# edsonportosilva/OptiCommPy

Hardware: AMD Instinct MI355X
Metric: SSFM steps/sec (2-pol, 2^20 samples) (higher is better)
Workload: dtype f64

## Files before the change

### opticommpy_amd/csrc/fused_engine.h

```cpp
#pragma once
#include <algorithm>
#include <cmath>
#include <cstdlib>
#include <cstring>
#include <memory>
#include <string>
#include <type_traits>
#include <vector>

#include "fused_kernels.h"
#include "ssf_derived.h"

namespace ssf {
namespace fused {

#ifndef SSF_EXPERIMENTS
#define SSF_EXPERIMENTS 0
#endif
static inline const char *tune_env(const char *name) {
#if SSF_EXPERIMENTS
    return std::getenv(name);
#else
    (void)name;
    return nullptr;
// ... 101 lines not shown
            if (force_c && C != force_c) continue;
            const size_t cl = mix2_col_lds(n1, C, 2, s), rl = 4096 + (size_t)n2 * s;
            if (cl > 156 * 1024) continue;
            double score = (cl <= 80 * 1024 ? 0.0 : 4.0) + ((rl <= 72 * 1024 && n2 <= 4096) ? 0.0 : 3.0) + (C == 8 ? 0.0 : C == 4 ? 1.0 : 3.0) +
                           0.5 * std::fabs(std::log2((double)n1 / 256.0));
            const double col_wgs = (double)((n2 + C - 1) / C), row_wgs = (2 * n1 >= 1024 && n2 <= 2048) ? (double)n1 : 2.0 * n1;
            score += 4.0 * std::max(0.0, std::log2(256.0 / col_wgs)) + 4.0 * std::max(0.0, std::log2(256.0 / row_wgs));
            MixPlan cp;
            const int tcol = 256 / (2 * C);
            if (mix_make_plan(n1, &cp, tcol, false))
                for (int i = 0; i < cp.npass; ++i) score += 0.5 * (double)((n1 / cp.r[i] + tcol - 1) / tcol - 1);
            if (score < best) {
                best = score;
                *N1o = n1;
                *N2o = (int)n2;
                *Co = C;
            }
        }
    }
    return best < 1e300;
}

static inline bool choose_nonpow2_split(int64_t N, int precision, int f1, int fc, bool l1_forced, int *l1, int *N1, int *N2, int *C) {
    *l1 = *N1 = *N2 = *C = 0;
    if (f1 > 0 && choose_mixed2_split(N, precision, N1, N2, C, f1, fc)) return true;
    if (!choose_mixed_split(N, precision, l1, N2)) {
        *l1 = *N2 = 0;
        return choose_mixed2_split(N, precision, N1, N2, C);
    }
    if (*l1 < 7 && !l1_forced) {
        int n1 = 0, n2 = 0, c = 0;
        if (choose_mixed2_split(N, precision, &n1, &n2, &c)) {
            *l1 = 0;
            *N1 = n1;
            *N2 = n2;
            *C = c;
        }
    }
    return true;
}

template <typename T, class Backend> class FusedCore {
  public:
    using C = cx<T>;
    using S = scalar_t<T>;
    static constexpr bool kPacked = sizeof(T) != sizeof(S);
    Backend &be;
    int64_t N;
    int nrows, log2N;
    Split sp;
    int N2mix = 0;
    int mix_rows = 1;
    MixPlan mix_plan{};
    cx<double> *wtab = nullptr;
    int N1mix = 0, mix_cols = 0;
    MixPlan mix_plan1{};
    cx<double> *wtab1 = nullptr;
    int n1() const { return N1mix ? N1mix : 1 << sp.l1; }
    int row_tw_off = 0;
    size_t field_bytes;
    C *G = nullptr, *T0 = nullptr, *T1 = nullptr, *Ehd = nullptr, *noise_d = nullptr;
    S *P = nullptr, *Theta = nullptr;
    bool own_G = true;
    void *cpl_comm = nullptr;
    double *cpl_work = nullptr;
    std::unique_ptr<FusedCore<pf2, Backend>> pk;
    bool use_packed = true;
    bool lim0_bound = true;
    Ctrl *ctrl = nullptr;
    LinOp *linops = nullptr;
    unsigned *gbar = nullptr;
    double *part = nullptr;
    double *tr_hz = nullptr, *tr_lim = nullptr;
    int *tr_it = nullptr;
    long long tr_cap = 0;
    int tr_maxIter = 0;
    std::vector<C *> snaps;
    int row_v = 16;
    int col_v = 16;
    bool underfilled = false;
    int lanes_hint = 1;
    int col_split = 1;
    int row_pair = -1;
    bool split_ok = true;
    int split_penalty = 0;
    static constexpr int kSplitPenalty = 8;
    int hint_n_it = 0;
    int cur = 0;
    unsigned seq = 0;
    int row_block, row_grid, col_block_mk, col_grid_mk, col_block_1, col_grid_1, npart_max;
    size_t row_lds, col_lds_mk, col_lds_1;
    std::string err;

    std::vector<ssf_stats> ustats;
    int units = 1;
    int npairs() const { return kPacked ? nrows : std::max(nrows / 2, 1); }
    int rows_u() const { return nrows / units; }
    int pairs_u() const { return std::max(npairs() / units, 1); }
    FusedCore(Backend &b, int64_t N_, int nrows_, int precision, void *borrowed_G = nullptr, int units_ = 1)
        : be(b), N(N_), nrows(nrows_), units(units_ > 0 ? units_ : 1) {
        if (borrowed_G) {
            G = (C *)borrowed_G;
            own_G = false;
        }
        log2N = 0;
        while ((1ll << log2N) < N) ++log2N;
        if ((N & (N - 1)) == 0) {
            choose_split(log2N, precision, &sp, kPacked);
        } else {
            sp.l1 = sp.l2 = 0;
            int f1 = 0, fc = 0;
            if (const char *e = tune_env("SSF_MIX2")) {
                f1 = std::atoi(e);
                if (const char *q = std::strchr(e, ',')) fc = std::atoi(q + 1);
            }
            if (!choose_nonpow2_split(N, precision, f1, fc, tune_env("SSF_MIX_L1") != nullptr, &sp.l1, &N1mix, &N2mix, &mix_cols))
                sp.l1 = N1mix = N2mix = mix_cols = 0;
        }
        field_bytes = sizeof(C) * (size_t)N * (size_t)nrows;
    }

    void col_geometry(int groups, int npol, int *block, int *grid, size_t *lds) const {
        if (N1mix) {
            *block = 256;
            *grid = groups * ((N2mix + mix_cols - 1) / mix_cols);
            *lds = mix2_col_lds(N1mix, mix_cols, npol, (int)sizeof(C));
            return;
        }
        const int tpf = (1 << sp.l1) / col_v, N2 = N2mix ? N2mix : 1 << sp.l2;
        int half = col_v == 8 ? 512 / npol : 256;
        if (const char *e = tune_env("SSF_COL_HALF")) {
            const int h = std::atoi(e);
            if (h >= tpf && h <= 512 && (h & (h - 1)) == 0) half = h;
        }
        while (half / tpf > N2 && half > tpf) half >>= 1;
        auto wgs = [&](int h) { return (long long)groups * (N2 / (h / tpf)); };
        while (!tune_env("SSF_COL_HALF") && half > 64 &&
               ((wgs(half) < 512 && (half / tpf) * sizeof(C) > 128) || (wgs(half) < 256 && (half / tpf) * sizeof(C) > 64)))
            half >>= 1;
        const int Cc = half / tpf;
        *block = half * npol;
        *grid = groups * ((N2 + Cc - 1) / Cc);
        *lds = std::max((size_t)npol * Cc * lds_col_stride(1 << sp.l1, Cc, (int)sizeof(C)) * sizeof(C), (size_t)half * npol * 16 + 1024);
    }

    int init() {
        if (const char *e = tune_env("SSF_LIM0_BOUND")) lim0_bound = std::atoi(e) != 0;
        if (const char *e = tune_env("SSF_COL_SPLIT")) col_split = std::atoi(e);
        if (const char *e = tune_env("SSF_ROW_PAIR")) row_pair = std::atoi(e) != 0;
        underfilled = (double)rows_u() * (double)N <= 1048576.0;
        col_v = underfilled && sp.l1 != 7 ? 8 : 16;
        if (const char *e = tune_env("SSF_COL_V")) col_v = std::atoi(e) == 8 ? 8 : 16;
        if (N2mix || sp.l1 < 6 || sp.l1 > 10) col_v = 16;
        if (N1mix && !mix_make_plan(N1mix, &mix_plan1, 256 / (2 * mix_cols), false)) {
            err = "fused engine: no pass plan for the column length";
            return SSF_ERR_UNSUPPORTED;
        }
        if (const char *e = N1mix ? tune_env("SSF_MIX_PLAN1") : nullptr) {
            int r[kMixMaxPass], n = 0;
            for (const char *q = e; *q && n < kMixMaxPass;) {
                r[n++] = std::atoi(q);
                while (*q && *q != ',') ++q;
                if (*q == ',') ++q;
            }
            MixPlan mp;
            if (mix_plan_from_radices(N1mix, r, n, &mp)) mix_plan1 = mp;
        }
        const int64_t nfft = (int64_t)rows_u() * n1();
        if (N2mix) {
            int tpr = 128;
            if (const char *e = tune_env("SSF_MIX_TPR")) tpr = std::max(64, std::min(1024, std::atoi(e)));
            while (16 * tpr < N2mix) tpr *= 2;
            mix_rows = std::max(1, 256 / tpr);
            while (nfft % mix_rows) mix_rows >>= 1;
            while (mix_rows > 1 && 4096 + (size_t)mix_rows * N2mix * sizeof(C) > 72 * 1024) mix_rows >>= 1;
            while (mix_rows > 1 && nfft / mix_rows < 512) {
                mix_rows >>= 1;
                tpr *= 2;
            }
            row_block = tpr * mix_rows;
            row_grid = (int)(nfft / mix_rows);
            row_lds = 4096 + (size_t)mix_rows * N2mix * sizeof(C);
            mix_make_plan(N2mix, &mix_plan, tpr);
            if (const char *e = tune_env("SSF_MIX_PLAN")) {
                int r[kMixMaxPass], n = 0;
                for (const char *q = e; *q && n < kMixMaxPass;) {
                    r[n++] = std::atoi(q);
                    while (*q && *q != ',') ++q;
                    if (*q == ',') ++q;
                }
                MixPlan mp;
                if (mix_plan_from_radices(N2mix, r, n, &mp) && mp.r[mp.npass - 1] <= kMixMaxOpRadix) mix_plan = mp;
            }
        } else {
            row_v = underfilled ? 8 : 16;
            if (const char *e = tune_env("SSF_ROW_V")) row_v = std::atoi(e) == 8 ? 8 : 16;
            if (sp.l2 < 6) row_v = 16;
            const int tpf2 = (1 << sp.l2) / row_v, wg = row_v == 8 ? 512 : 256;
            int fpw = tpf2 >= wg ? 1 : wg / tpf2;
            if (underfilled && row_v == 8) fpw = units > 1 ? std::max(1, std::min(fpw, 256 / std::max(tpf2, 1))) : 1;
            if (const char *e = tune_env("SSF_ROW_FPW")) fpw = std::max(1, std::min(fpw, std::atoi(e)));
            while (nfft % fpw) fpw >>= 1;
            row_block = fpw * tpf2;
            row_grid = (int)(nfft / fpw);
            row_lds = std::max((size_t)fpw * lds_slots_per_fft(1 << sp.l2) * sizeof(C), (size_t)row_block * 16 + 2048);
            if ((SSF_TW_TAB & 1) && sizeof(S) == 4) {
                row_tw_off = (int)((row_lds + 15) / 16 * 16);
                row_lds = (size_t)row_tw_off + kTwLdsBytes;
            }
        }
        if (const char *e = std::getenv("SSF_C64_PACKED")) use_packed = std::atoi(e) != 0;
        col_geometry(pairs_u(), kPacked ? 1 : 2, &col_block_mk, &col_grid_mk, &col_lds_mk);
        col_geometry(rows_u(), 1, &col_block_1, &col_grid_1, &col_lds_1);
        npart_max = std::max(col_grid_mk, col_grid_1);
        if (own_G && !(G = (C *)be.alloc(field_bytes))) return oom();
        if (!(T0 = (C *)be.alloc(field_bytes))) return oom();
        if (kPacked && mk_buffers()) return SSF_ERR_OOM;
        if (!(ctrl = (Ctrl *)be.alloc(2 * (size_t)units * sizeof(Ctrl)))) return oom();
        if (!(linops = (LinOp *)be.alloc(2 * sizeof(LinOp)))) return oom();
        if (!(gbar = (unsigned *)be.alloc(8 * sizeof(unsigned)))) return oom();
        if (!(part = (double *)be.alloc(sizeof(double) * 5 * (size_t)units * (size_t)npart_max))) return oom();
        if (N2mix) {
            if (!(wtab = (cx<double> *)be.alloc(sizeof(cx<double>) * (size_t)N2mix))) return oom();
            std::vector<cx<double>> w((size_t)N2mix);
            for (int q = 0; q < N2mix; ++q) {
                const double a = -2.0 * 3.14159265358979323846 * (double)q / (double)N2mix;
                w[(size_t)q].re = std::cos(a);
                w[(size_t)q].im = std::sin(a);
            }
            be.h2d(wtab, w.data(), sizeof(cx<double>) * (size_t)N2mix);
        }
        if (N1mix) {
// ... 254 lines not shown
                    a.bar = gbar;
                    int rc = be.launch_nlse_span(a, pgrid, plds);
                    if (rc) return hiperr();
                }
            } else if (nsteps >= 1) {
                launch_col_plain(CM_NLSE_FIRST, E, (S)0);
                launch_row_lin(linops + 0);
                for (int s = 1; s < nsteps; ++s) {
                    launch_col_plain(CM_NLSE_STEP, E, (S)(p.gamma * p.hz));
                    launch_row_lin(linops + 1);
                }
                launch_col_plain(CM_NLSE_STEP, E, (S)(p.gamma * p.hz));
                launch_row_lin(linops + 0);
                launch_col_plain(CM_NLSE_LAST, E, (S)0);
            }
            int rc = amp_fwd(p, d, span, span - s0, noise, std::exp(d.alpha_lin / 2 * nsteps * p.hz));
            if (rc) return rc;
            if (wants_snapshot(p, span) && (rc = snapshot())) return rc;
            st->steps += nsteps;
            st->transforms += (int64_t)nrows * (2 * (int64_t)nsteps + 2);
        }
        be.sync();
        if (pgrid > 0) {
            unsigned flags[3] = {0, 0, 0};
            be.d2h(flags, gbar, sizeof(flags));
            if (flags[2]) {
                err = "persistent span kernel: grid barrier timed out (workgroups not co-resident?)";
                return SSF_ERR_STATE;
            }
        }
        return be.ok() ? SSF_OK : hiperr();
    }

    MkConst mk_const(const ssf_params &p, const Derived &d) const {
        MkConst k{};
        k.Lspan = p.Lspan;
        k.hz_fixed = p.hz;
        k.tol = p.tol;
        k.maxRot = p.maxNlinPhaseRot;
        k.c8g = d.c8g;
        k.sgn = p.direction >= 0 ? 1.0 : -1.0;
        k.lin_a = d.lin_a;
        k.lin_b = d.lin_b;
        k.w2 = (d.w_scale / (double)N) * (d.w_scale / (double)N);
        k.invN = 1.0 / (double)N;
        k.maxIter = p.maxIter;
        k.adaptive = p.nlprMethod ? 1 : 0;
        k.exact_lim0 = (p.maxIter == 1 || !lim0_bound) ? 1 : 0;
        k.log2N = log2N;
        k.trace_cap = tr_cap;
        k.tr_hz = tr_hz;
        k.tr_it = tr_it;
        k.tr_lim = tr_lim;
        return k;
    }
    void launch_mk_row(const MkConst &k, bool pair = false) {
        RowArgs<T> a = row_args();
        a.use_ctrl = 1;
        a.pair = pair ? 1 : 0;
        a.cin = ctrl + (size_t)(seq & 1) * units;
        a.cout = ctrl + (size_t)((seq + 1) & 1) * units;
        a.k = k;
        const size_t ps = (size_t)units * (size_t)npart_max;
        a.pmax = part;
        a.pnum = part + ps;
        a.pden = part + 2 * ps;
        a.pnum0 = part + 3 * ps;
        a.pden0 = part + 4 * ps;
        a.npart = col_grid_mk;
        if constexpr (Backend::kCanCouple) {
            if (cpl_comm) {
                if (be.couple(cpl_comm, part, ps, col_grid_mk, cpl_work)) return;
                a.pnum0 = cpl_work;
                a.pden0 = cpl_work + 1;
                a.pnum = cpl_work + 2;
                a.pden = cpl_work + 3;
                a.pmax = cpl_work + 4;
                a.npart = 1;
            }
        }
        be.launch_row(a, row_grid, row_block, row_lds, units);
        ++seq;
    }
    void launch_mk_col(const MkConst &k, int mode, int sg = SG_ALL) {
        ColArgs<T> a = col_args(kPacked ? 1 : 2, mode);
        a.sg = sg;
        a.cin = ctrl + (size_t)(seq & 1) * units;
        a.cout = ctrl + (size_t)((seq + 1) & 1) * units;
        a.k = k;
        a.npart = col_grid_mk;
        be.launch_col(a, col_grid_mk, col_block_mk, col_lds_mk, units);
        ++seq;
    }
    int prepare_trace(ssf_trace *trace, int maxIter) {
        const long long cap = trace ? trace->capacity : 0;
        if (cap > tr_cap || maxIter != tr_maxIter) {
            for (void *q : {(void *)tr_hz, (void *)tr_lim, (void *)tr_it})
                if (q) be.free(q);
            tr_hz = tr_lim = nullptr;
            tr_it = nullptr;
            tr_cap = 0;
            if (cap > 0) {
                tr_hz = (double *)be.alloc(sizeof(double) * (size_t)cap);
                tr_it = (int *)be.alloc(sizeof(int) * (size_t)cap);
                tr_lim = (double *)be.alloc(sizeof(double) * (size_t)cap * (size_t)maxIter);
                if (!tr_hz || !tr_it || !tr_lim) return oom();
                tr_cap = cap;
                tr_maxIter = maxIter;
            }
        }
        if (tr_cap > 0) be.memset(tr_lim, 0xFF, sizeof(double) * (size_t)tr_cap * (size_t)maxIter);
        return SSF_OK;
    }

    struct SpanRun {
        long long trace_n = 0;
        double avg_it = 3.0;
        int n_it = 0;
    };
    int run_span(const ssf_params &p, const MkConst &k, SpanRun &sr, ssf_stats *st) {
        std::vector<Ctrl> cs((size_t)units);
        for (auto &c : cs) {
            c = Ctrl{};
            c.state = ST_NEED_S;
            c.cur = cur;
            c.trace_n = sr.trace_n;
        }
        const size_t cbytes = sizeof(Ctrl) * (size_t)units;
        be.h2d(ctrl + (size_t)(seq & 1) * units, cs.data(), cbytes);
        bool persisted = false;
        if constexpr (Backend::kCanPersist && !kPacked) {
            const int workers = be.persist_mk_workers();
            if (workers > 0 && units == 1 && !N2mix && row_block == 256 && col_block_mk == 256 && row_v == 16 && col_v == 16 &&
                std::is_same<T, double>::value) {
                SpanMkArgs<T> a{};
                a.row = row_args();
                a.row.use_ctrl = 1;
                a.row.k = k;
                a.row.pmax = part;
                a.row.pnum = part + npart_max;
                a.row.pden = part + 2 * (size_t)npart_max;
                a.row.pnum0 = part + 3 * (size_t)npart_max;
                a.row.pden0 = part + 4 * (size_t)npart_max;
                a.row.npart = col_grid_mk;
                a.col = col_args(2, CM_MK);
                a.row.tw_off = 0;
                a.col.k = k;
                a.col.npart = col_grid_mk;
                a.ctrl = ctrl;
                a.seq0 = seq;
                a.row_grid = row_grid;
                a.col_grid = col_grid_mk;
                a.max_stages = 1 << 20;
                a.nworkers = std::min(workers, std::max(row_grid, col_grid_mk));
                a.xcd = be.persist_mk_xcd() ? 0 : -1;
                a.ctrl_lds = (std::max(row_lds, col_lds_mk) + 15) / 16 * 16;
                a.bar = gbar;
                const int grid = a.xcd >= 0 ? 8 * a.nworkers : a.nworkers;
                if (be.launch_mk_span(a, grid, a.ctrl_lds + sizeof(Ctrl) + 64)) return hiperr();
                unsigned flags[8] = {0, 0, 0, 0, 0, 0, 0, 0};
                be.d2h(flags, gbar, sizeof(flags));
                if (!be.ok()) return hiperr();
                if (flags[2]) {
                    err = "persistent Manakov kernel: grid barrier timed out (workgroups not co-resident / not on one XCD?)";
                    return SSF_ERR_STATE;
                }
                seq = (seq & ~1u) | (flags[4] & 1u);
                be.d2h(cs.data(), ctrl + (seq & 1), sizeof(Ctrl));
                if (!be.ok()) return hiperr();
                if (cs[0].state != ST_SPAN_DONE || cs[0].pend0) {
                    err = "persistent Manakov kernel: span not finished";
                    return SSF_ERR_STATE;
                }
                persisted = true;
            }
        }
        if (!persisted) {
        launch_mk_col(k, CM_MK);
        int guard = 0;
        long long prev_steps = 0, prev_iters = 0, prev_rare = 0;
        const bool can_split = col_split && split_penalty == 0 && units == 1 && !cpl_comm &&
                               be.can_split_cols(col_args(kPacked ? 1 : 2, CM_MK), col_block_mk);
        bool general_chunk = false;
        int stalls = 0, pos = 0;
        const bool can_pair = can_split && units == 1 && std::is_same<T, double>::value && !N1mix && !N2mix && row_v == 16 && !p.nlprMethod &&
                              PairRows<Backend>::ok(be, sp.l2, row_block) && (row_pair < 0 ? !underfilled : row_pair != 0);
        bool skip_row = false;
        double z_sim = 0.0;
        long long idle_pairs = 0;
        for (;;) {
            double steps_rem = 0.0;
            for (const Ctrl &c : cs) {
                double r;
                if (c.state == ST_SPAN_DONE && !c.pend0) r = 0.0;
                else if (c.steps == 0 && c.state == ST_NEED_S) r = p.nlprMethod ? 8.0 : std::ceil(p.Lspan / p.hz);
                else r = std::max(1.0, std::ceil((p.Lspan - c.z) / (c.hz > 0 ? c.hz : p.hz)));
                steps_rem = std::max(steps_rem, r);
            }
            const bool use_split = can_split && split_ok && !general_chunk;
            const int n_pred = std::max(1, std::min(p.maxIter, sr.n_it > 0 ? sr.n_it : (int)std::lround(sr.avg_it)));
            double est = p.nlprMethod ? steps_rem * (1.0 + sr.avg_it) * 0.6
                                      : steps_rem * (1.0 + (use_split ? std::max((double)n_pred, sr.avg_it) : sr.avg_it)) + 3.0;
            int chunk = (int)std::min(512.0, std::max(2.0, std::ceil(est)));
            if (can_split && split_ok && general_chunk) chunk = std::min(chunk, 8);
            else if (use_split && sr.n_it == 0) chunk = std::min(chunk, 4 * (n_pred + 1));
            const bool pairing = use_split && can_pair;
            z_sim = cs[0].z;
            skip_row = pairing && pos == 0 && cs[0].state == ST_NEED_H;
            for (int i = 0; i < chunk; ++i) {
                if (!(pairing && pos == 0 && skip_row)) launch_mk_row(k, pairing);
                int sg = SG_ALL;
                if (use_split) {
                    sg = pos == 0 ? (SG_H | SG_RARE) : pos < n_pred ? SG_ADV : SG_FIN;
                    if (pairing && pos >= n_pred) {
                        const double hz_sim = pick_hz(k, z_sim, 0.0);
                        skip_row = z_sim + hz_sim < k.Lspan && pick_hz(k, z_sim + hz_sim, 0.0) == hz_sim;
                        z_sim += hz_sim;
                    }
                    pos = pos >= n_pred ? 0 : pos + 1;
                }
                launch_mk_col(k, CM_MK, sg);
            }
            be.d2h(cs.data(), ctrl + (size_t)(seq & 1) * units, cbytes);
            if (!be.ok()) return hiperr();
            long long steps = 0, iters = 0, rare = 0;
            bool done = true;
            double worst = 0.0;
            for (const Ctrl &c : cs) {
                steps += c.steps;
                iters += c.iterations;
                rare += c.n_rebuilt + c.n_recovered;
                done = done && c.state == ST_SPAN_DONE && !c.pend0;
                if (c.steps > 0) worst = std::max(worst, (double)c.iterations / (double)c.steps);
            }
            if (steps > prev_steps) {
                sr.avg_it = units == 1 ? (double)(iters - prev_iters) / (double)(steps - prev_steps) : worst;
                sr.n_it = cs[0].last_nit;
            }
            if (can_split && split_ok && !done) {
                idle_pairs = steps == prev_steps ? idle_pairs + chunk : 0;
                const bool stuck = idle_pairs >= 2 * (n_pred + 1) + 2;
                if (general_chunk && !stuck) general_chunk = false;
                else if (stuck) {
                    general_chunk = true;
                    if (++stalls >= 2) split_ok = false;
                }
                if (rare - prev_rare > (steps - prev_steps) / 4 + 2) split_ok = false;
                if (!split_ok) split_penalty = kSplitPenalty;
            }
            prev_steps = steps;
            prev_iters = iters;
            prev_rare = rare;
            if (done) break;
            if (++guard > (1 << 22)) {
                err = "fused engine: span did not terminate";
                return SSF_ERR_STATE;
            }
        }
        }
        if (units == 1) {
            cur = cs[0].cur;
        } else {
            const size_t ub = sizeof(C) * (size_t)rows_u() * (size_t)N;
            for (int u = 0; u < units; ++u)
                if (cs[(size_t)u].cur != cur)
                    be.d2d((char *)(cur ? T1 : T0) + (size_t)u * ub, (char *)(cur ? T0 : T1) + (size_t)u * ub, ub);
        }
        sr.trace_n = cs[0].trace_n;
        if ((int)ustats.size() != units) ustats.assign((size_t)units, ssf_stats{});
        for (int u = 0; u < units; ++u) {
            const Ctrl &c = cs[(size_t)u];
            ssf_stats &us = ustats[(size_t)u];
            us.steps += c.steps;
            us.iterations += c.iterations;
            us.nonconverged_steps += c.nonconv;
            us.decided_ahead += c.n_ahead;
            us.rebuilt_iterates += c.n_rebuilt;
            us.recovered_fields += c.n_recovered;
            us.transforms += (int64_t)(kPacked ? 2 * rows_u() : rows_u()) * (2 * c.steps + 2 * c.iterations);
        }
        for (const Ctrl &c : cs) {
            st->steps += c.steps;
            st->iterations += c.iterations;
            st->nonconverged_steps += c.nonconv;
            st->decided_ahead += c.n_ahead;
            st->rebuilt_iterates += c.n_rebuilt;
            st->recovered_fields += c.n_recovered;
            st->transforms += (int64_t)(kPacked ? 2 * rows_u() : rows_u()) * (2 * c.steps + 2 * c.iterations);
        }
        return SSF_OK;
    }
    int fetch_trace(ssf_trace *trace, long long trace_n, int maxIter) {
        if (trace) {
            trace->count = trace_n;
            const long long n = std::min(trace_n, (long long)trace->capacity);
            if (n > 0) {
                if (trace->hz) be.d2h(trace->hz, tr_hz, sizeof(double) * (size_t)n);
                if (trace->iters) be.d2h(trace->iters, tr_it, sizeof(int) * (size_t)n);
                if (trace->lims) be.d2h(trace->lims, tr_lim, sizeof(double) * (size_t)n * (size_t)maxIter);
            }
        }
        return be.ok() ? SSF_OK : hiperr();
    }
    MkConst mk_const_for(const ssf_params &p, const Derived &d, ssf_trace *trace) const {
// ... 123 lines not shown
```

### opticommpy_amd/csrc/fused_kernels.h

```cpp
#pragma once
#include "fused_core.h"
#include "mixed_fft.h"
#include "ssf_rng.h"

namespace ssf {
namespace fused {

enum {
    ST_NEED_S = 0,
    ST_AFTER_S = 1,
    ST_NEED_H = 2,
    ST_ROW_ITER = 3,
    ST_NEED_I = 4,
    ST_SPAN_DONE = 6,
    ST_REDO0 = 7,
    ST_RECOVER_A = 8,
    ST_RECOVER_ROW = 9,
    ST_RECOVER_B = 10
};

struct LinOp {
    double cth;
    double mag;
    double Cre[9], Cim[9];
// ... 836 lines not shown
            }
            if (lin16) lb = lin16_bases<V>(cth_pre, k1r + ((long long)rev_pos(p, reg_pos(p, last, br, 0)) << a.log2N1), log2N);
            ctx.issue_fence();
        }
#endif
        fft_dif<-1, V, kTab>(ctx, p, br, v, l, tws);
        ctx.mark(2);
        if (a.prio) ctx.template setprio<1>();
        if (!a.use_ctrl && !a.lin) {
            if (a.fwd_only) {
#pragma unroll
                for (int idx = 0; idx < V; ++idx) g[reg_pos(p, last, br, idx)] = v[idx];
                return;
            }
            const cx<T> *h = a.harr + ((size_t)k1r << a.log2N2);
#pragma unroll
            for (int idx = 0; idx < V; ++idx) v[idx] = v[idx] * h[reg_pos(p, last, br, idx)];
        } else if (p.lg(last) == lgV) {
#if SSF_EARLY_BASES
            if (lo.cth != lb.cth) lb = lin16_bases<V>(lo.cth, k1r + ((long long)rev_pos(p, reg_pos(p, last, br, 0)) << a.log2N1), log2N);
            apply_lin16<V>(lo, lb, v);
#else
            if constexpr (kPair) apply_lin16<V>(lo, lbr, v);
            else {
                const long long k0 = k1r + ((long long)rev_pos(p, reg_pos(p, last, br, 0)) << a.log2N1);
                apply_lin16<V>(lo, k0, log2N, v);
            }
#endif
        } else {
#pragma unroll
            for (int idx = 0; idx < V; ++idx) {
                const long long k = k1r + ((long long)rev_pos(p, reg_pos(p, last, br, idx)) << a.log2N1);
                v[idx] = mul_by_d(v[idx], lin_at(lo, k, log2N));
            }
        }
        ctx.mark(3);
        fft_dit<+1, V, kTab>(ctx, p, br, v, l, tws);
        if (a.prio) ctx.template setprio<0>();
        ctx.mark(4);
        row_store<V>(ctx, a, gdst, p, fr, br, v);
        if constexpr (!kPair) break;
        else {
            if (round || !rp.on) break;
            lo = a.cin->lin;
            lo.mag *= (double)row_n1(a);
            uniform_linop(lo);
            gdst = a.G;
        }
    }
    ctx.mark(5);
    ctx.flush(0);
}

enum {
    CM_NLSE_FIRST = 0,
    CM_NLSE_STEP = 1,
    CM_NLSE_LAST = 2,
    CM_MK = 3,
    CM_PLAIN_FWD = 5,
    CM_PLAIN_INV = 6
};

template <typename T> struct ColArgs {
    cx<T> *G;
    cx<T> *T0, *T1;
    cx<T> *Ehd;
    scalar_t<T> *P;
    scalar_t<T> *Theta;
    int log2N1, log2N2, npol, mode;
    int ngroups;
    scalar_t<T> g_hz;
    const Ctrl *cin;
    Ctrl *cout;
    MkConst k;
    double *pmax, *pnum, *pden, *pnum0, *pden0;
    int npart;
    int N2;
    long long N;
    int vpt;
    long long u_elems;
    int u_part;
    int prio;
    int sg;
    int N1mix, mix_cols;
    MixPlan plan1;
    const cx<double> *wtab1;
};

template <typename T> SSF_HD RowArgs<T> unit_view(const RowArgs<T> &a, int u) {
    RowArgs<T> b = a;
    b.G += (long long)u * a.u_elems;
    if (a.cin) b.cin += u;
    if (a.cout) b.cout += u;
    const long long po = (long long)u * a.u_part;
    if (a.pmax) b.pmax += po;
    if (a.pnum) b.pnum += po;
    if (a.pden) b.pden += po;
    if (a.pnum0) b.pnum0 += po;
    if (a.pden0) b.pden0 += po;
    return b;
}
template <typename T> SSF_HD ColArgs<T> unit_view(const ColArgs<T> &a, int u) {
    ColArgs<T> b = a;
    if (u > 0) {
        const long long fo = (long long)u * a.u_elems;
        b.G += fo;
        if (a.T0) b.T0 += fo;
        if (a.T1) b.T1 += fo;
        if (a.Ehd) b.Ehd += fo;
        const long long N = a.N2 ? a.N : 1ll << (a.log2N1 + a.log2N2);
        if (a.P) b.P += 2 * N * a.ngroups * (long long)u;
        if (a.Theta) b.Theta += N * a.ngroups * (long long)u;
        if (a.cin) b.cin += u;
        if (a.cout) b.cout += u;
        const long long po = (long long)u * a.u_part;
        if (a.pmax) b.pmax += po;
        if (a.pnum) b.pnum += po;
        if (a.pden) b.pden += po;
        if (a.pnum0) b.pnum0 += po;
        if (a.pden0) b.pden0 += po;
    }
    return b;
}

template <typename T, int LG, class Ctx, bool RAGGED = false, int V = 16> struct ColGeom {
    static constexpr int kV = V;
    static constexpr bool kDppT = SSF_PAIR_DPP && V == 16 && sizeof(T) == 8;
    bool dpp;
    PassPlan p;
    int half, pol, t, C, c, b, n2, N2;
    bool valid;
    long long N;
    long long rowbase;
    long long pbase;
    SSF_HD ColGeom(Ctx &ctx, const ColArgs<T> &a) {
        p = make_plan(LG > 0 ? LG : a.log2N1, V == 16 ? 4 : 3);
        half = ctx.nthreads / a.npol;
        dpp = kDppT && a.npol == 2;
        if (kDppT && a.npol == 2) {
            pol = ctx.tid & 1;
            t = ctx.tid >> 1;
        } else {
            pol = ctx.tid / half;
            t = ctx.tid - pol * half;
        }
        C = half / p.tpf;
        c = t % C;
        b = t / C;
        N2 = RAGGED ? a.N2 : 1 << a.log2N2;
        const int tpp = RAGGED ? (N2 + C - 1) / C : N2 / C;
        const int grp = ctx.bid / tpp;
        int tile = ctx.bid - grp * tpp;
        if (tpp % 8 == 0) tile = (tile & 7) * (tpp >> 3) + (tile >> 3);
        else if (RAGGED && tpp > 8) {
            const int q = tpp >> 3, r = tpp & 7, x = tile & 7;
            tile = x * q + (x < r ? x : r) + (tile >> 3);
        }
        n2 = tile * C + c;
        valid = !RAGGED || n2 < N2;
        N = RAGGED ? a.N : 1ll << (a.log2N1 + a.log2N2);
        rowbase = (long long)(grp * a.npol + pol) * N;
        pbase = (long long)grp * N;
    }
    SSF_HD long long freq_off(int q) const { return (long long)(b + p.tpf * q) * N2 + n2; }
    SSF_HD long long time_off(int idx) const {
        return (long long)rev_pos(p, reg_pos(p, p.npass - 1, b, idx)) * N2 + n2;
// ... 21 lines not shown
            w0 = cis2pi<double>((double)SIGN * ((double)(((long long)g.n2 * g.b) % g.N) / (double)g.N));
            ws = cis2pi<double>((double)SIGN * ((double)(((long long)g.n2 * g.p.tpf) % g.N) / (double)g.N));
        } else {
            const long long N = 1ll << log2N;
            w0 = cis2pi<double>((double)SIGN * scale_pow2((double)(((long long)g.n2 * g.b) & (N - 1)), log2N));
            ws = cis2pi<double>((double)SIGN * scale_pow2((double)(((long long)g.n2 * g.p.tpf) & (N - 1)), log2N));
        }
        if (SSF_TW_REUSE) {
            gt.w0 = SIGN > 0 ? w0 : conj(w0);
            gt.ws = SIGN > 0 ? ws : conj(ws);
            gt.have = true;
        }
    }
    constexpr int V = G::kV;
    cx<double> t[V];
    const cx<double> s2 = ws * ws, s4 = s2 * s2;
    t[0] = w0;
    t[1] = w0 * ws;
    t[2] = t[0] * s2;
    t[3] = t[1] * s2;
#pragma unroll
    for (int q = 0; q < 4; ++q) t[4 + q] = t[q] * s4;
    if constexpr (V == 16) {
        const cx<double> s8 = s4 * s4;
#pragma unroll
        for (int q = 0; q < 8; ++q) t[8 + q] = t[q] * s8;
    }
#pragma unroll
    for (int q = 0; q < V; ++q) v[q] = mul_by_d(v[q], t[q]);
}

template <typename U, class Ctx, class G> SSF_HD void pair_swap(Ctx &ctx, const G &g, const U *mine, U *other, U *sh) {
    constexpr int V = G::kV;
    if constexpr (G::kDppT) {
        if (g.dpp) {
#pragma unroll
            for (int idx = 0; idx < V; ++idx) other[idx] = (U)ctx.xchg((double)mine[idx]);
            return;
        }
    }
#pragma unroll
    for (int idx = 0; idx < V; ++idx) sh[(size_t)(g.pol * V + idx) * g.half + g.t] = mine[idx];
    ctx.sync();
#pragma unroll
    for (int idx = 0; idx < V; ++idx) other[idx] = sh[(size_t)((g.pol ^ 1) * V + idx) * g.half + g.t];
}

template <class G> SSF_HD int own_idx(const G &g, int j) { return g.pol ? j + G::kV / 2 : j; }
template <class G> SSF_HD int oth_idx(const G &g, int j) { return g.pol ? j : j + G::kV / 2; }
template <class G> SSF_HD long long own_time_off(const G &g, int j) { return g.pol ? g.time_off(j + G::kV / 2) : g.time_off(j); }
template <typename U, class G> SSF_HD U pick16(const G &g, int idx, const U *own, const U *oth) {
    constexpr int H = G::kV / 2;
    return ((idx / H) == g.pol) ? own[idx % H] : oth[idx % H];
}

template <typename T, class Ctx, class G>
SSF_HD void pair_cis(Ctx &ctx, const G &g, const T *ang_own, cx<T> *rot, cx<T> *sh) {
    constexpr int V = G::kV, H = V / 2;
    cx<T> own[H], oth[H];
    if constexpr (G::kDppT) {
        if (g.dpp) {
#pragma unroll
            for (int j = 0; j < H; ++j) {
                own[j] = cis_t<T>(ang_own[j]);
                oth[j] = mk<T>((T)ctx.xchg((double)own[j].re), (T)ctx.xchg((double)own[j].im));
            }
#pragma unroll
            for (int idx = 0; idx < V; ++idx) rot[idx] = pick16(g, idx, own, oth);
            return;
        }
    }
#pragma unroll
    for (int j = 0; j < H; ++j) {
        own[j] = cis_t<T>(ang_own[j]);
        sh[(size_t)own_idx(g, j) * g.half + g.t] = own[j];
    }
    ctx.sync();
#pragma unroll
    for (int j = 0; j < H; ++j) oth[j] = sh[(size_t)oth_idx(g, j) * g.half + g.t];
#pragma unroll
    for (int idx = 0; idx < V; ++idx) rot[idx] = pick16(g, idx, own, oth);
}

template <typename T, class Ctx, class G>
SSF_HD void mk_step_start(Ctx &ctx, const G &g, const ColArgs<T> &a, const cx<T> *v, T *Pbuf, bool lds_busy) {
    constexpr int V = G::kV;
    T *shT = (T *)ctx.lds;
    T mine[V], oth[V];
#pragma unroll
    for (int idx = 0; idx < V; ++idx) mine[idx] = norm2(v[idx]);
    if (lds_busy && !(G::kDppT && g.dpp)) ctx.sync();
    pair_swap(ctx, g, mine, oth, shT);
    const T c8g = (T)a.k.c8g;
    double m = -INFINITY;
#pragma unroll
    for (int idx = 0; idx < V; ++idx) {
        const T ax = g.pol ? oth[idx] : mine[idx], ay = g.pol ? mine[idx] : oth[idx];
        const T pw = ax + ay;
        if (g.pol == 0) g.st(Pbuf, g.pbase + g.time_off(idx), pw);
        const T phi = c8g * (pw + ax + ay) / (T)2;
        m = (double)phi > m ? (double)phi : m;
    }
    if (a.k.adaptive) {
        m = block_max(ctx, m, (double *)ctx.lds);
        if (ctx.tid == 0) a.pmax[ctx.bid] = m;
    }
    ctx.sync();
}
template <typename T, class G> SSF_HD T theta_ld(const G &g, const T *th, long long i) {
    if constexpr (SSF_THETA_F32 && sizeof(T) == 8) return (T)g.ld((const float *)th, i);
    else return g.ld(th, i);
}
template <typename T, class G> SSF_HD void theta_st(const G &g, T *th, long long i, T x) {
    if constexpr (SSF_THETA_F32 && sizeof(T) == 8) g.st((float *)th, i, (float)x);
    else g.st(th, i, x);
}
template <typename T, class Ctx, class G>
SSF_HD void mk_advance_dpp(Ctx &ctx, const G &g, const ColArgs<T> &a, cx<T> *v, const T *Pbuf, T shz, bool first,
                           double &num, double &den, double &pch_sum) {
    constexpr int V = G::kV, H = V / 2;
    T pw8[H], prev8[H], ang8[H];
#pragma unroll
    for (int j = 0; j < H; ++j) {
        const long long t = own_time_off(g, j);
        pw8[j] = g.ld(Pbuf, g.pbase + t);
        prev8[j] = first ? (T)0 : theta_ld(g, a.Theta, g.pbase + t);
    }
    const T c8g = (T)a.k.c8g;
#pragma unroll
    for (int j = 0; j < H; ++j) {
        const T lo = norm2(v[j]), hi = norm2(v[j + H]);
        const T nown = g.pol ? hi : lo, noth = g.pol ? lo : hi;
        const T po = (T)ctx.xchg((double)noth);
        const T ax = g.pol ? po : nown, ay = g.pol ? nown : po;
        const T pw = pw8[j];
        pch_sum += (double)pw;
        ang8[j] = shz * (c8g * (pw + ax + ay) / (T)2);
        if (first) prev8[j] = shz * (c8g * (pw + pw) / (T)2);
    }
    ctx.mark(6);
#pragma unroll
    for (int idx = 0; idx < V; ++idx) v[idx] = g.ld(a.Ehd, g.rowbase + g.time_off(idx));
    ctx.mark(7);
#pragma unroll
    for (int j = 0; j < H; ++j) {
        const T ang = ang8[j];
        const double s = sin_half_angle((double)ang - (double)prev8[j]);
        theta_st(g, a.Theta, g.pbase + own_time_off(g, j), ang);
        const cx<T> ro = cis_t<T>(ang);
        const T dd = (T)(4.0 * s * s);
        const cx<T> rp = mk<T>((T)ctx.xchg((double)ro.re), (T)ctx.xchg((double)ro.im));
        const T dp = (T)ctx.xchg((double)dd);
        const cx<T> r_lo = g.pol ? rp : ro, r_hi = g.pol ? ro : rp;
        const T d_lo = g.pol ? dp : dd, d_hi = g.pol ? dd : dp;
        const double w0 = (double)norm2(v[j]), w1 = (double)norm2(v[j + H]);
        num += w0 * (double)d_lo + w1 * (double)d_hi;
        den += w0 + w1;
        v[j] = v[j] * r_lo;
        v[j + H] = v[j + H] * r_hi;
    }
}
template <typename T, class Ctx, class G>
SSF_HD void mk_advance(Ctx &ctx, const G &g, const ColArgs<T> &a, cx<T> *v, const T *Pbuf, T shz, bool first,
                       double &num, double &den, double &pch_sum) {
    constexpr int V = G::kV, H = V / 2;
    T *shN = (T *)ctx.lds;
    cx<T> *shC = (cx<T> *)(shN + V * (size_t)g.half);
    T *shD = (T *)(shC + V * (size_t)g.half);
    T nown[H], noth[H];
    T pw8[H], prev8[H];
#pragma unroll
    for (int j = 0; j < H; ++j) {
        const long long t = own_time_off(g, j);
        pw8[j] = g.ld(Pbuf, g.pbase + t);
        prev8[j] = first ? (T)0 : theta_ld(g, a.Theta, g.pbase + t);
    }
#pragma unroll
    for (int j = 0; j < H; ++j) {
        const T lo = norm2(v[j]), hi = norm2(v[j + H]);
        nown[j] = g.pol ? hi : lo;
        noth[j] = g.pol ? lo : hi;
    }
    ctx.sync();
#pragma unroll
    for (int j = 0; j < H; ++j) shN[(size_t)oth_idx(g, j) * g.half + g.t] = noth[j];
    ctx.sync();
    const T c8g = (T)a.k.c8g;
    T ang8[H];
#pragma unroll
    for (int j = 0; j < H; ++j) {
        const T po = shN[(size_t)own_idx(g, j) * g.half + g.t];
        const T ax = g.pol ? po : nown[j], ay = g.pol ? nown[j] : po;
        const T pw = pw8[j];
        pch_sum += (double)pw;
        ang8[j] = shz * (c8g * (pw + ax + ay) / (T)2);
        if (first) prev8[j] = shz * (c8g * (pw + pw) / (T)2);
    }
    ctx.mark(6);
#pragma unroll
    for (int idx = 0; idx < H; ++idx) v[idx] = g.ld(a.Ehd, g.rowbase + g.time_off(idx));
#pragma unroll
    for (int j = 0; j < H; ++j) {
        const long long t = own_time_off(g, j);
        const T ang = ang8[j], prev = prev8[j];
        const double s = sin_half_angle((double)ang - (double)prev);
        theta_st(g, a.Theta, g.pbase + t, ang);
        shC[(size_t)own_idx(g, j) * g.half + g.t] = cis_t<T>(ang);
        shD[(size_t)own_idx(g, j) * g.half + g.t] = (T)(4.0 * s * s);
    }
    ctx.mark(7);
#pragma unroll
    for (int idx = H; idx < V; ++idx) v[idx] = g.ld(a.Ehd, g.rowbase + g.time_off(idx));
    ctx.sync();
#pragma unroll
    for (int idx = 0; idx < V; ++idx) {
        const cx<T> e = v[idx];
        const double w = (double)norm2(e);
        num += w * (double)shD[(size_t)idx * g.half + g.t];
        den += w;
        v[idx] = e * shC[(size_t)idx * g.half + g.t];
    }
    ctx.sync();
}

struct MkColStage {
    bool do_inv = false, do_fwd = false, final_ = false, more = false, exact0 = true;
    bool sparse = false;
    bool paired = false;
    int op = -1;
    struct { int state, it, cur, pcur; double z, hz; } c{};
};
template <int V> SSF_HD bool lim0_bound_sample(int idx, int b) { return idx == 0 && (V == 16 || !(b & 1)); }
enum { SG_H = 1, SG_ADV = 2, SG_FIN = 4, SG_RARE = 8, SG_ALL = 15 };
SSF_HD int stage_group(int op, bool final_) { return op == 1 ? SG_H : op == 2 ? (final_ ? SG_FIN : SG_ADV) : SG_RARE; }
template <class Ctx, class Args> SSF_HD void mk_col_stage(Ctx &ctx, const Args &a, MkColStage &st, int sg_mask = SG_ALL) {
    bool &do_inv = st.do_inv, &do_fwd = st.do_fwd, &final_ = st.final_, &more = st.more, &exact0 = st.exact0;
    int &op = st.op;
    auto &c = st.c;
    c.state = a.cin->state;
    c.it = a.cin->it;
    c.cur = a.cin->cur;
    c.pcur = a.cin->pcur;
    c.z = a.cin->z;
    c.hz = a.cin->hz;
    final_ = a.cin->final_ != 0;
    exact0 = a.k.exact_lim0 || a.cin->exact0 != 0;
    const int c_exact0 = a.cin->exact0, c_redo = a.cin->redo_;
    const bool c_paired = a.cin->final_ == kFinalPaired;
    const long long c_trace_n = a.cin->trace_n, c_steps = a.cin->steps, c_iters = a.cin->iterations;
    const long long c_rebuilt = a.cin->n_rebuilt, c_recovered = a.cin->n_recovered;
    if (c.state == ST_NEED_S) {
        op = 0;
        do_fwd = true;
    } else if (c.state == ST_NEED_H) {
        op = 1;
        do_inv = do_fwd = true;
    } else if (c.state == ST_NEED_I) {
        op = 2;
        do_inv = true;
        more = c.z + c.hz < a.k.Lspan;
        do_fwd = final_ ? false : true;
        st.sparse = final_ && more && !a.k.exact_lim0 && !a.cin->dense &&
                    (a.k.adaptive || pick_hz(a.k, c.z + c.hz, 0.0) == c.hz);
        st.paired = more && c_paired;
    } else if (c.state == ST_REDO0) {
        op = 3;
        do_fwd = true;
    } else if (c.state == ST_RECOVER_A) {
        op = 4;
        do_fwd = true;
    } else if (c.state == ST_RECOVER_B) {
        op = 5;
        do_inv = do_fwd = true;
    }
    if (op >= 0 && !(stage_group(op, final_) & sg_mask)) {
        op = -1;
        do_inv = do_fwd = false;
    }
    if (ctx.bid == 0 && ctx.tid == 0) {
        ctrl_forward(a.cin, a.cout, (int)(sizeof(Ctrl) / 8));
        Ctrl *n = a.cout;
        if (op == 0) {
            n->state = ST_AFTER_S;
            n->gscale = 0;
            n->t_sparse = n->dense = 0;
            n->hz_valid = 0;
        } else if (op == 1) {
            n->state = ST_ROW_ITER;
            n->it = 0;
            n->final_ = a.k.maxIter == 1;
            n->pendn = 0;
        } else if (op == 4) {
            n->state = ST_RECOVER_ROW;
        } else if (op == 3 || op == 5) {
            if (op == 5) n->t_sparse = 0;
            n->state = ST_ROW_ITER;
            n->it = 0;
            n->final_ = c_exact0 ? 0 : 1;
            n->redo_ = c_exact0 ? 0 : 1;
            n->pend0 = n->pendn = 0;
            n->n_rebuilt = c_rebuilt + 1;
            if (op == 5) n->n_recovered = c_recovered + 1;
        } else if (op == 2 && !final_) {
            n->state = ST_ROW_ITER;
            n->it = c.it + 1;
            n->pendn = 1;
            if (c.it == 0) {
                n->pend0 = 1;
                n->pend0_idx = c_trace_n;
                n->bound0 = exact0 ? 0 : 1;
                n->exact0 = 0;
            }
        } else if (op == 2) {
            const long long tn = c_trace_n;
            if (tn < a.k.trace_cap) {
                if (a.k.tr_hz) a.k.tr_hz[tn] = c.hz;
                if (a.k.tr_it) a.k.tr_it[tn] = c.it + 1;
            }
            n->trace_n = tn + 1;
            n->steps = c_steps + 1;
            n->iterations = c_iters + c.it + 1;
            n->last_nit = c.it + 1;
            n->z = c.z + c.hz;
            n->cur = c.cur ^ 1;
            n->it = 0;
            n->final_ = 0;
            if (c.it == 0) {
                n->pend0 = 1;
                n->pend0_idx = tn;
                n->cap0 = c_redo ? 0 : 1;
                n->bound0 = exact0 ? 0 : 1;
                n->exact0 = 0;
            }
            n->redo_ = 0;
            n->t_sparse = st.sparse ? 1 : 0;
            n->dense = 0;
            if (more) {
                n->gscale = st.paired ? 0 : 1;
                n->state = st.paired ? ST_NEED_H : ST_AFTER_S;
                n->pcur = c.pcur ^ 1;
                if (a.k.adaptive) n->hz_valid = 0;
                else {
                    const double hz = pick_hz(a.k, c.z + c.hz, 0.0);
                    if (hz != c.hz) n->hz_valid = 0;
                    n->hz = hz;
                }
            } else n->state = ST_SPAN_DONE;
        }
    }
}

#define G_DPP(g) (std::remove_reference<decltype(g)>::type::kDppT && (g).dpp)
template <typename T, int LG, int MODE, bool RAGGED, int V = 16, int CI = 0, int SG = SG_ALL, class Ctx>
SSF_HD void col_body(Ctx &ctx, const ColArgs<T> &a) {
    constexpr int H = V / 2;
    constexpr int kCI = CI > 0 ? CI : 1;
    constexpr bool kMk = MODE == CM_MK;
    constexpr bool kgH = (SG & SG_H) != 0, kgADV = (SG & SG_ADV) != 0, kgFIN = (SG & SG_FIN) != 0, kgRARE = (SG & SG_RARE) != 0;
    constexpr bool kFwd = !kMk || kgH || kgADV || kgRARE;
    bool do_inv = false, do_fwd = false;
    int op = -1;
    bool final_ = false, more = false, exact0 = true, sparse = false, paired = false;
    struct { int state, it, cur, pcur; double z, hz; } c{};
    double *red = (double *)ctx.lds;
    ctx.mark(0);
    ColGeom<T, LG, Ctx, RAGGED, V> g(ctx, a);
    cx<T> v[V];
#if SSF_SPEC_G
    if (kMk) {
#pragma unroll
        for (int q = 0; q < V; ++q) {
            v[q] = g.ld(a.G, g.rowbase + g.freq_off(q));
            if ((q & 3) == 3) ctx.issue_fence();
        }
    }
#endif
    if (kMk) {
        MkColStage st;
        mk_col_stage(ctx, a, st, SG);
        do_inv = st.do_inv;
        do_fwd = kFwd && st.do_fwd;
        final_ = kgFIN && (!kgADV || st.final_);
        more = st.more;
        exact0 = st.exact0;
        sparse = st.sparse;
        paired = kgFIN && st.paired;
        op = st.op;
        c.state = st.c.state;
        c.it = st.c.it;
        c.cur = st.c.cur;
        c.pcur = st.c.pcur;
        c.z = st.c.z;
        c.hz = st.c.hz;
        if (op < 0) return;
    } else {
        do_inv = MODE == CM_NLSE_STEP || MODE == CM_NLSE_LAST || MODE == CM_PLAIN_INV;
        do_fwd = MODE == CM_NLSE_STEP || MODE == CM_NLSE_FIRST || MODE == CM_PLAIN_FWD;
    }

    const PassPlan &p = g.p;
    cx<T> *lds = CI > 0 ? (cx<T> *)ctx.lds + (size_t)g.pol * CI * lds_slots_per_fft(p.L) + g.c
                        : (cx<T> *)ctx.lds + (size_t)(g.pol * g.C + g.c) * lds_col_stride(p.L, g.C, (int)sizeof(cx<T>));

    cx<T> *Tcur = a.T0, *Tnew = a.T1;
    T *Pcur = a.P, *Palt = a.P;
    if (kMk) {
        Tcur = c.cur ? a.T1 : a.T0;
        Tnew = c.cur ? a.T0 : a.T1;
        const long long psz = g.N * a.ngroups;
        Pcur = a.P + (c.pcur ? psz : 0);
        Palt = a.P + (c.pcur ? 0 : psz);
    }

    TwSrc<T> tws;
    GTw gtw;
    cx<T> e_pre{};
    if (do_inv) {
        if (!(kMk && SSF_SPEC_G)) {
            auto load_spectrum = [&](const cx<T> *Gin) {
#pragma unroll
                for (int q = 0; q < V; ++q) {
                    v[q] = g.ld(Gin, g.rowbase + g.freq_off(q));
#if SSF_LOAD_ORDER
                    if ((q & 3) == 3) ctx.issue_fence();
#endif
                }
            };
            if constexpr (kMk && kgFIN) load_spectrum(paired ? Tnew : a.G);
            else load_spectrum(a.G);
        }
        if (kMk && (kgADV || kgFIN) && op == 2 && c.it == 0 && !exact0 && lim0_bound_sample<V>(0, g.b)) e_pre = g.ld(Tcur, g.rowbase + g.time_off(0));
        ctx.mark(1);
        if (a.prio) ctx.template setprio<3>();
        global_twiddle<+1, RAGGED>(g, a.log2N1 + a.log2N2, v, gtw);
        fft_dif<+1, V, false, kCI>(ctx, p, g.b, v, lds, tws);
        ctx.mark(2);
        if (a.prio) ctx.template setprio<2>();
    } else if (kMk && !kgRARE) {
    } else if (!(kMk && op == 3)) {
        const cx<T> *src = kMk && op == 4 ? a.Ehd : Tcur;
#pragma unroll
        for (int idx = 0; idx < V; ++idx) v[idx] = g.ld(src, g.rowbase + g.time_off(idx));
    }

    if (MODE == CM_NLSE_STEP) {
#pragma unroll
        for (int idx = 0; idx < V; ++idx) v[idx] = v[idx] * cis_t<T>(a.g_hz * norm2(v[idx]));
    } else if (MODE == CM_NLSE_LAST || MODE == CM_PLAIN_INV) {
#pragma unroll
        for (int idx = 0; idx < V; ++idx) g.st(a.T0, g.rowbase + g.time_off(idx), v[idx]);
    } else if (kMk) {
        const T shz = (T)(a.k.sgn * c.hz), c8g = (T)a.k.c8g;
        cx<T> *shC = (cx<T> *)(ctx.lds + 2 * V * (size_t)g.half * sizeof(T));
        if (kgRARE && op == 0) {
            mk_step_start(ctx, g, a, v, Pcur, false);
        } else if (kgRARE && op == 4) {
        } else if ((kgH && op == 1) || (kgRARE && (op == 3 || op == 5))) {
            T ang[H];
#pragma unroll
            for (int j = 0; j < H; ++j) {
                const T pw = g.ld(Pcur, g.pbase + own_time_off(g, j));
                ang[j] = shz * (c8g * (pw + pw) / (T)2);
            }
#pragma unroll
            for (int idx = 0; idx < V; ++idx) {
                const long long t = g.time_off(idx);
                if (!kgRARE || op == 1) g.st(a.Ehd, g.rowbase + t, v[idx]);
                else {
                    if (op == 5) g.st(Tcur, g.rowbase + t, v[idx]);
                    v[idx] = g.ld(a.Ehd, g.rowbase + t);
                }
            }
            cx<T> rot[V];
            if (!G_DPP(g)) ctx.sync();
            pair_cis(ctx, g, ang, rot, shC);
#pragma unroll
            for (int idx = 0; idx < V; ++idx) v[idx] = v[idx] * rot[idx];
            ctx.sync();
        } else if (kgADV || kgFIN) {
            double n0 = 0, d0 = 0, n1 = 0, d1 = 0, psum = 0;
            if (c.it == 0) {
                cx<T> e[V];
                if (exact0) {
#pragma unroll
                    for (int idx = 0; idx < V; ++idx) e[idx] = g.ld(Tcur, g.rowbase + g.time_off(idx));
                } else e[0] = e_pre;
#pragma unroll
                for (int idx = 0; idx < V; ++idx) {
                    if (exact0 || lim0_bound_sample<V>(idx, g.b)) {
                        const double dr = (double)v[idx].re - (double)e[idx].re, di = (double)v[idx].im - (double)e[idx].im;
                        n0 += dr * dr + di * di;
                        d0 += (double)e[idx].re * e[idx].re + (double)e[idx].im * e[idx].im;
                    }
                }
            }
            if (final_) {
#pragma unroll
                for (int idx = 0; idx < V; ++idx)
                    if (!sparse || lim0_bound_sample<V>(idx, g.b)) g.st(Tnew, g.rowbase + g.time_off(idx), v[idx]);
            } else if (kgADV) {
                if (G_DPP(g)) mk_advance_dpp(ctx, g, a, v, Pcur, shz, c.it == 0, n1, d1, psum);
                else mk_advance(ctx, g, a, v, Pcur, shz, c.it == 0, n1, d1, psum);
                if (!exact0) d0 = psum;
            }
            if (c.it == 0) {
                block_sum2(ctx, n0, d0, red);
                if (ctx.tid == 0) {
                    a.pnum0[ctx.bid] = n0;
                    a.pden0[ctx.bid] = d0;
                }
            }
            if (!final_) {
                block_sum2(ctx, n1, d1, red);
                if (ctx.tid == 0) {
                    a.pnum[ctx.bid] = n1;
                    a.pden[ctx.bid] = d1;
                }
                ctx.sync();
            } else if (more) {
                mk_step_start(ctx, g, a, v, Palt, true);
            }
        }
    }

    ctx.mark(3);
    if (a.prio) ctx.template setprio<1>();
    if (kFwd && do_fwd) {
        if (!kMk && do_inv) ctx.sync();
        fft_dit<-1, V, false, kCI>(ctx, p, g.b, v, lds, tws);
        global_twiddle<-1, RAGGED>(g, a.log2N1 + a.log2N2, v, gtw);
        ctx.mark(4);
        if (a.prio) ctx.template setprio<0>();
#pragma unroll
        for (int q = 0; q < V; ++q) g.st(a.G, g.rowbase + g.freq_off(q), v[q]);
        ctx.mark(5);
        ctx.flush(do_inv ? 0 : 1);
    }
}

constexpr int kColMixScratch = 8192;
constexpr int kMix2MaxCol = 1024;
template <typename T, int MODE, class Ctx> SSF_HD void col_mixed_body(Ctx &ctx, const ColArgs<T> &a, const MixPlan &plan1) {
    static_assert(sizeof(T) == sizeof(scalar_t<T>), "one row per polarisation (no packed pairs)");
    constexpr bool kMk = MODE == CM_MK;
// ... 680 lines not shown
```

Before: 6539.

## Chain final column stage with next step's half-step kernel to skip a launch

Adds a chained column mode for the Manakov solver. When the step size is unchanged and rows are paired, the final (FIN) column pass of one step and the H stage of the next step run in a single launch. The power values are kept in registers instead of being reloaded, and the control state is advanced directly to the row-iteration state. This removes one kernel launch and one global round-trip of the power buffer per step. In exchange it adds a new kernel variant with more register pressure and more complex control-state handoff.

```diff
diff --git a/opticommpy_amd/csrc/fused_engine.h b/opticommpy_amd/csrc/fused_engine.h
--- a/opticommpy_amd/csrc/fused_engine.h
+++ b/opticommpy_amd/csrc/fused_engine.h
@@ -207,6 +207,7 @@
     int lanes_hint = 1;
     int col_split = 1;
     int row_pair = -1;
+    int col_chain = -1;
     bool split_ok = true;
     int split_penalty = 0;
     static constexpr int kSplitPenalty = 8;
@@ -273,6 +274,7 @@
         if (const char *e = tune_env("SSF_LIM0_BOUND")) lim0_bound = std::atoi(e) != 0;
         if (const char *e = tune_env("SSF_COL_SPLIT")) col_split = std::atoi(e);
         if (const char *e = tune_env("SSF_ROW_PAIR")) row_pair = std::atoi(e) != 0;
+        if (const char *e = tune_env("SSF_COL_CHAIN")) col_chain = std::atoi(e) != 0;
         underfilled = (double)rows_u() * (double)N <= 1048576.0;
         col_v = underfilled && sp.l1 != 7 ? 8 : 16;
         if (const char *e = tune_env("SSF_COL_V")) col_v = std::atoi(e) == 8 ? 8 : 16;
@@ -693,9 +695,10 @@
         be.launch_row(a, row_grid, row_block, row_lds, units);
         ++seq;
     }
-    void launch_mk_col(const MkConst &k, int mode, int sg = SG_ALL) {
+    void launch_mk_col(const MkConst &k, int mode, int sg = SG_ALL, bool chain = false) {
         ColArgs<T> a = col_args(kPacked ? 1 : 2, mode);
         a.sg = sg;
+        a.chain = chain ? 1 : 0;
         a.cin = ctrl + (size_t)(seq & 1) * units;
         a.cout = ctrl + (size_t)((seq + 1) & 1) * units;
         a.k = k;
@@ -796,7 +799,9 @@
         int stalls = 0, pos = 0;
         const bool can_pair = can_split && units == 1 && std::is_same<T, double>::value && !N1mix && !N2mix && row_v == 16 && !p.nlprMethod &&
                               PairRows<Backend>::ok(be, sp.l2, row_block) && (row_pair < 0 ? !underfilled : row_pair != 0);
+        const bool can_chain = can_pair && (col_chain < 0 ? !underfilled : col_chain != 0);
         bool skip_row = false;
+        bool skip_h = false;
         double z_sim = 0.0;
         long long idle_pairs = 0;
         for (;;) {
@@ -817,20 +822,32 @@
             else if (use_split && sr.n_it == 0) chunk = std::min(chunk, 4 * (n_pred + 1));
             const bool pairing = use_split && can_pair;
             z_sim = cs[0].z;
+            const bool chaining = pairing && can_chain;
             skip_row = pairing && pos == 0 && cs[0].state == ST_NEED_H;
+            skip_h = chaining && pos == 0 && cs[0].state == ST_ROW_ITER && cs[0].it == 0;
             for (int i = 0; i < chunk; ++i) {
+                if (chaining && pos == 0 && skip_h) {
+                    skip_h = false;
+                    pos = pos >= n_pred ? 0 : pos + 1;
+                    continue;
+                }
                 if (!(pairing && pos == 0 && skip_row)) launch_mk_row(k, pairing);
                 int sg = SG_ALL;
+                bool chain = false;
                 if (use_split) {
                     sg = pos == 0 ? (SG_H | SG_RARE) : pos < n_pred ? SG_ADV : SG_FIN;
                     if (pairing && pos >= n_pred) {
                         const double hz_sim = pick_hz(k, z_sim, 0.0);
                         skip_row = z_sim + hz_sim < k.Lspan && pick_hz(k, z_sim + hz_sim, 0.0) == hz_sim;
                         z_sim += hz_sim;
+                        if (chaining && skip_row) {
+                            sg = SG_H | SG_RARE;
+                            chain = skip_h = true;
+                        }
                     }
                     pos = pos >= n_pred ? 0 : pos + 1;
                 }
-                launch_mk_col(k, CM_MK, sg);
+                launch_mk_col(k, CM_MK, sg, chain);
             }
             be.d2h(cs.data(), ctrl + (size_t)(seq & 1) * units, cbytes);
             if (!be.ok()) return hiperr();
diff --git a/opticommpy_amd/csrc/fused_kernels.h b/opticommpy_amd/csrc/fused_kernels.h
--- a/opticommpy_amd/csrc/fused_kernels.h
+++ b/opticommpy_amd/csrc/fused_kernels.h
@@ -942,6 +942,7 @@
     int u_part;
     int prio;
     int sg;
+    int chain;
     int N1mix, mix_cols;
     MixPlan plan1;
     const cx<double> *wtab1;
@@ -1129,13 +1130,20 @@
     for (int idx = 0; idx < V; ++idx) rot[idx] = pick16(g, idx, own, oth);
 }
 
-template <typename T, class Ctx, class G>
-SSF_HD void mk_step_start(Ctx &ctx, const G &g, const ColArgs<T> &a, const cx<T> *v, T *Pbuf, bool lds_busy) {
+template <typename T> SSF_HD T norm2_pinned(cx<T> a) {
+#if defined(__HIP_DEVICE_COMPILE__)
+    if constexpr (std::is_same<T, double>::value) return __builtin_fma(a.im, a.im, a.re * a.re);
+    else
+#endif
+        return norm2(a);
+}
+template <bool MAXPHI = true, typename T, class Ctx, class G>
+SSF_HD void mk_step_start(Ctx &ctx, const G &g, const ColArgs<T> &a, const cx<T> *v, T *Pbuf, bool lds_busy, T *pw_out = nullptr) {
     constexpr int V = G::kV;
     T *shT = (T *)ctx.lds;
     T mine[V], oth[V];
 #pragma unroll
-    for (int idx = 0; idx < V; ++idx) mine[idx] = norm2(v[idx]);
+    for (int idx = 0; idx < V; ++idx) mine[idx] = norm2_pinned(v[idx]);
     if (lds_busy && !(G::kDppT && g.dpp)) ctx.sync();
     pair_swap(ctx, g, mine, oth, shT);
     const T c8g = (T)a.k.c8g;
@@ -1145,10 +1153,13 @@
         const T ax = g.pol ? oth[idx] : mine[idx], ay = g.pol ? mine[idx] : oth[idx];
         const T pw = ax + ay;
         if (g.pol == 0) g.st(Pbuf, g.pbase + g.time_off(idx), pw);
-        const T phi = c8g * (pw + ax + ay) / (T)2;
-        m = (double)phi > m ? (double)phi : m;
-    }
-    if (a.k.adaptive) {
+        if (pw_out) pw_out[idx] = pw;
+        if constexpr (MAXPHI) {
+            const T phi = c8g * (pw + ax + ay) / (T)2;
+            m = (double)phi > m ? (double)phi : m;
+        }
+    }
+    if (MAXPHI && a.k.adaptive) {
         m = block_max(ctx, m, (double *)ctx.lds);
         if (ctx.tid == 0) a.pmax[ctx.bid] = m;
     }
@@ -1274,6 +1285,8 @@
     bool do_inv = false, do_fwd = false, final_ = false, more = false, exact0 = true;
     bool sparse = false;
     bool paired = false;
+    bool chain_kernel = false;
+    bool chain = false;
     int op = -1;
     struct { int state, it, cur, pcur; double z, hz; } c{};
 };
@@ -1325,7 +1338,8 @@
         do_inv = do_fwd = false;
     }
     if (ctx.bid == 0 && ctx.tid == 0) {
-        ctrl_forward(a.cin, a.cout, (int)(sizeof(Ctrl) / 8));
+        const Ctrl *fsrc = st.chain_kernel ? (const Ctrl *)((const char *)a.cin + opaque_i(0)) : a.cin;
+        ctrl_forward(fsrc, a.cout, (int)(sizeof(Ctrl) / 8));
         Ctrl *n = a.cout;
         if (op == 0) {
             n->state = ST_AFTER_S;
@@ -1392,6 +1406,11 @@
                     if (hz != c.hz) n->hz_valid = 0;
                     n->hz = hz;
                 }
+                if (st.chain && st.paired) {
+                    n->state = ST_ROW_ITER;
+                    n->final_ = a.k.maxIter == 1;
+                    n->pendn = 0;
+                }
             } else n->state = ST_SPAN_DONE;
         }
     }
@@ -1405,9 +1424,11 @@
     constexpr bool kMk = MODE == CM_MK;
     constexpr bool kgH = (SG & SG_H) != 0, kgADV = (SG & SG_ADV) != 0, kgFIN = (SG & SG_FIN) != 0, kgRARE = (SG & SG_RARE) != 0;
     constexpr bool kFwd = !kMk || kgH || kgADV || kgRARE;
+    constexpr bool kChain = kMk && SG == (SG_H | SG_RARE) && V == 16 && sizeof(T) == 8 && !RAGGED && CI == 0 && !SSF_SPEC_G;
     bool do_inv = false, do_fwd = false;
     int op = -1;
     bool final_ = false, more = false, exact0 = true, sparse = false, paired = false;
+    bool st_paired = false;
     struct { int state, it, cur, pcur; double z, hz; } c{};
     double *red = (double *)ctx.lds;
     ctx.mark(0);
@@ -1424,7 +1445,11 @@
 #endif
     if (kMk) {
         MkColStage st;
-        mk_col_stage(ctx, a, st, SG);
+        if constexpr (kChain) {
+            st.chain_kernel = true;
+            st.chain = a.chain != 0 && !a.k.adaptive;
+            mk_col_stage(ctx, a, st, st.chain ? (SG | SG_FIN) : SG);
+        } else mk_col_stage(ctx, a, st, SG);
         do_inv = st.do_inv;
         do_fwd = kFwd && st.do_fwd;
         final_ = kgFIN && (!kgADV || st.final_);
@@ -1432,6 +1457,7 @@
         exact0 = st.exact0;
         sparse = st.sparse;
         paired = kgFIN && st.paired;
+        st_paired = kChain && st.paired;
         op = st.op;
         c.state = st.c.state;
         c.it = st.c.it;
@@ -1459,6 +1485,70 @@
         Palt = a.P + (c.pcur ? 0 : psz);
     }
 
+    T pk[kChain ? H : 1];
+    bool pk_valid = false;
+    if constexpr (kChain) {
+        if (op == 2) {
+            const cx<T> *Gin = st_paired ? Tnew : a.G;
+#pragma unroll
+            for (int q = 0; q < V; ++q) {
+                v[q] = g.ld(Gin, g.rowbase + g.freq_off(q));
+#if SSF_LOAD_ORDER
+                if ((q & 3) == 3) ctx.issue_fence();
+#endif
+            }
+            cx<T> e[V];
+            if (c.it == 0 && !exact0 && lim0_bound_sample<V>(0, g.b)) e[0] = g.ld(Tcur, g.rowbase + g.time_off(0));
+            if (a.prio) ctx.template setprio<3>();
+            {
+                TwSrc<T> tw1;
+                GTw gt1;
+                ColGeom<T, LG, Ctx, RAGGED, V> g1 = g;
+                g1.b = opaque_i(g.b);
+                g1.n2 = opaque_i(g.n2);
+                global_twiddle<+1, RAGGED>(g1, a.log2N1 + a.log2N2, v, gt1);
+                fft_dif<+1, V, false, kCI>(ctx, g1.p, g1.b, v, lds, tw1);
+            }
+            if (a.prio) ctx.template setprio<2>();
+            if (c.it == 0) {
+                double n0 = 0, d0 = 0;
+                if (exact0) {
+#pragma unroll
+                    for (int idx = 0; idx < V; ++idx) e[idx] = g.ld(Tcur, g.rowbase + g.time_off(idx));
+                }
+#pragma unroll
+                for (int idx = 0; idx < V; ++idx) {
+                    if (exact0 || lim0_bound_sample<V>(idx, g.b)) {
+                        const double dr = (double)v[idx].re - (double)e[idx].re, di = (double)v[idx].im - (double)e[idx].im;
+                        n0 += dr * dr + di * di;
+                        d0 += (double)e[idx].re * e[idx].re + (double)e[idx].im * e[idx].im;
+                    }
+                }
+#pragma unroll
+                for (int idx = 0; idx < V; ++idx)
+                    if (!sparse || lim0_bound_sample<V>(idx, g.b)) g.st(Tnew, g.rowbase + g.time_off(idx), v[idx]);
+                block_sum2(ctx, n0, d0, red);
+                if (ctx.tid == 0) {
+                    a.pnum0[ctx.bid] = n0;
+                    a.pden0[ctx.bid] = d0;
+                }
+            } else {
+#pragma unroll
+                for (int idx = 0; idx < V; ++idx)
+                    if (!sparse || lim0_bound_sample<V>(idx, g.b)) g.st(Tnew, g.rowbase + g.time_off(idx), v[idx]);
+            }
+            if (!more) return;
+            T pw[V];
+            mk_step_start<false>(ctx, g, a, v, Palt, true, pw);
+            if (!(a.chain && st_paired)) return;
+#pragma unroll
+            for (int j = 0; j < H; ++j) pk[j] = g.pol ? pw[j + H] : pw[j];
+            pk_valid = true;
+            op = 1;
+            do_inv = do_fwd = true;
+        }
+    }
+
     TwSrc<T> tws;
     GTw gtw;
     cx<T> e_pre{};
@@ -1506,7 +1596,7 @@
             T ang[H];
 #pragma unroll
             for (int j = 0; j < H; ++j) {
-                const T pw = g.ld(Pcur, g.pbase + own_time_off(g, j));
+                const T pw = kChain && pk_valid ? pk[j] : g.ld(Pcur, g.pbase + own_time_off(g, j));
                 ang[j] = shz * (c8g * (pw + pw) / (T)2);
             }
 #pragma unroll
```

New measurement: 6679 (median of 6 runs). 1.02x the previous value.
